# deepsound-project/pggan-pytorch

Hardware: AMD Instinct MI355X
Metric: images/sec, PGGAN full train step (D+GP step + G step + Adam) at 1024x1024 (higher is better)
Workload: dtype f32; 1 GPU; BASELINE config 5: PGGAN 1024x1024 net (fmap_base 4096, C=3, latent 512), stage depth 8 = 1024x1024, alpha 1.00, minibatch 3/GPU (reference schedule), Trainer.train(): WGAN-GP + Adam(0,0.99) at lr 0, fp32; resolution=1024, depth=8, minibatch_per_gpu=3, global_batch=3, parallelism=dp1, fmap_base=4096, hip_graphs=False

## Files before the change

pggan-pytorch_amd/csrc/conv_strip.hip:

```cpp
#include "convp.h"

#ifndef PG_STRIP_ABL
#define PG_STRIP_ABL 0
#endif

namespace {

using pgk::ConvP;
using pgk::pg_sign_byte;
using pgk::pg_sign_factors;
using pgk::g_last_kernel; using pgk::set_smem; using pgk::SMEM_ANY;

constexpr int SW = 64;
constexpr int RP = SW + 2;
constexpr int RB = 4;
constexpr int NBLK = 3;

enum { EPI_GENERIC = 0, EPI_FWD = 1, EPI_MASK = 2, EPI_PN = 3, EPI_PNB = 4 };

struct SArgs {
    const float* x; const float* w; const float* bias; const void* mask; float* y;
    unsigned char* ysigns; float* pn_r; const float* pnb_y; const float* pnb_r; float* ypool; const float* pool_other;
    float scale, slope, mask_slope, pn_eps, pool_a, pool_b;
    int H, W, ups, mask_bytes, y_bytes, pool_only;
    int strips, segs, seg_rows;
    const unsigned char* gbytes; float gmul, gslope;
    const float* rgb_w; const float* rgb_b; float rgb_scale, rgb_slope; int rgbC; unsigned char* xsigns;
    float* t_out; const float* t_w; const float* t_b; float t_scale; int tC, t_sc, t_sco, t_only;
    const float* fw_img; float* fw_dw; float* fw_db; float fw_scale;
};

template <int CIN> struct Blk {
    static constexpr int C4 = CIN / 4;
    static constexpr int USED = C4 * RB * RP;
    static constexpr int NWI = (USED + 63) / 64;
    static constexpr int NI = (NWI + 3) / 4;
    static constexpr int SLOTS = NWI * 64;
};

typedef __attribute__((address_space(3))) const char* lds_cptr;
typedef __attribute__((address_space(3))) const f32x4* lds_v4ptr;

__device__ __forceinline__ pg_u32x4 rsrc_words(const void* base, unsigned bytes)
{
    const unsigned long long a = (unsigned long long)base;
    return pg_u32x4{(unsigned)__builtin_amdgcn_readfirstlane((int)(unsigned)a),
                    (unsigned)__builtin_amdgcn_readfirstlane((int)((unsigned)(a >> 32) & 0xffffu)), bytes, 0x00020000u};
}
__device__ __forceinline__ void buf_store4(__amdgpu_buffer_rsrc_t r, unsigned voff, float4 v)
{
    __builtin_amdgcn_raw_buffer_store_b128(pg_u32x4{__float_as_uint(v.x), __float_as_uint(v.y), __float_as_uint(v.z), __float_as_uint(v.w)},
                                           r, (int)voff, 0, 0);
}

constexpr int RGB_MAXC = 3;
template <int COUT, int CIN, int EPI, bool WREG, int GM, int XM = 0>
__device__ __forceinline__ void conv_strip_body(const SArgs& p)
{
    constexpr bool GATH = GM != 0;
    using B = Blk<CIN>;
    constexpr int C4 = B::C4;
    constexpr int QO = COUT / 4, QP = 16 / QO, PXG = 4 * QP;
    constexpr int GPR = 32 / PXG, G = 2 * GPR;
    constexpr int BLKB = B::SLOTS * 16;
    constexpr bool GEN = EPI == EPI_GENERIC;
    extern __shared__ __align__(16) float lds[];
    constexpr int WS = CIN == 16 ? CIN + 4 : CIN;
    float* wl = lds + NBLK * B::SLOTS * 4;
    const int tid = threadIdx.x, lane = tid & 63, wave = __builtin_amdgcn_readfirstlane(tid >> 6);
    const int blk = lane >> 2, j = lane & 3, qo = blk % QO, qp = blk / QO;

    int t = (int)pg_xcd_remap(blockIdx.x, gridDim.x);
    const int strip = __builtin_amdgcn_readfirstlane(t % p.strips); t /= p.strips;
    const int seg = __builtin_amdgcn_readfirstlane(t % p.segs), n = __builtin_amdgcn_readfirstlane(t / p.segs);
    const int r0 = seg * p.seg_rows, ow0 = strip * SW;
    const int niter = p.seg_rows / RB;
    const int xH = p.ups ? (p.H >> 1) : p.H, xW = p.ups ? (p.W >> 1) : p.W;
    const unsigned npix = (unsigned)(p.H * p.W);

    const unsigned rowbytes = 4u * (unsigned)(xW * CIN);
    unsigned voff[B::NI], vstep[B::NI];
    const unsigned blkstep = (p.ups ? 2u : 4u) * rowbytes;
#pragma unroll
    for (int i = 0; i < B::NI; ++i) {
        const int sl = (i * 4 + wave) * 64 + lane;
        const int q = sl / (RB * RP), rem = sl - q * (RB * RP);
        const int m = rem / RP, px = rem - m * RP;
        const int col = ow0 - 1 + px, row = r0 - 1 + m;
        const bool ok = sl < B::USED && (unsigned)col < (unsigned)p.W;
        voff[i] = ok ? (unsigned)(p.ups ? (row >> 1) : row) * rowbytes + 4u * (unsigned)((p.ups ? (col >> 1) : col) * CIN + 4 * q) : PG_OOB;
        vstep[i] = ok ? blkstep : 0u;
    }
    const size_t ximg = (size_t)xH * xW * CIN;
    const pg_u32x4 rxs = rsrc_words(p.x + (size_t)n * ximg, (unsigned)(ximg * 4));
    const unsigned lds0 = (unsigned)(size_t)(__attribute__((address_space(3))) char*)lds;
    const unsigned wdst = __builtin_amdgcn_readfirstlane(lds0 + (unsigned)wave * 1024u);
    auto dma16 = [&](unsigned vo, unsigned dst) {
        unsigned keep;
        asm volatile("s_mov_b32 %0, m0\n\ts_mov_b32 m0, %3\n\ts_nop 0\n\tbuffer_load_dwordx4 %1, %2, 0 offen lds\n\ts_mov_b32 m0, %0"
                     : "=&s"(keep) : "v"(vo), "s"(rxs), "s"(dst) : "memory");
    };
    auto issue_block = [&](int pos) {
#pragma unroll
        for (int i = 0; i < B::NI; ++i) {
            if (i * 4 + wave < B::NWI) dma16(voff[i], wdst + (unsigned)pos * BLKB + (unsigned)i * 4096u);
            voff[i] += vstep[i];
        }
    };

    constexpr int NG = GATH ? (B::USED + 255) / 256 : 1;
    unsigned cvo[NG], cvs[NG], bvo[NG], bvs[NG];
    float4 gxr[NG];
    unsigned gbr[NG];
    __amdgpu_buffer_rsrc_t rgx = pg_make_rsrc(p.x + (size_t)n * ximg, (unsigned)(ximg * 4)), rgb = rgx;
    constexpr int NR = GM == 2 ? NG : 1;
    int rrow[NR];
    float rw[NR][4][RGB_MAXC], rb[NR][4], rpx[NR][RGB_MAXC];
    if constexpr (GM == 2) {
        rgx = pg_make_rsrc(p.x + (size_t)n * npix * p.rgbC, npix * (unsigned)p.rgbC * 4u);
        rgb = pg_make_rsrc(p.xsigns + (size_t)n * npix * C4, npix * C4);
#pragma unroll
        for (int i = 0; i < NG; ++i) {
            const int sl = i * 256 + tid;
            const int q = sl / (RB * RP), rem = sl - q * (RB * RP);
            const int m = rem / RP, px = rem - m * RP;
            const int col = ow0 - 1 + px;
            const bool ok = sl < B::USED && (unsigned)col < (unsigned)p.W;
            rrow[i] = ok ? r0 - 1 + m : -(1 << 28);
            cvo[i] = ok ? 4u * (unsigned)((r0 - 1 + m) * p.W + col) : PG_OOB;
            cvs[i] = ok ? 4u * (unsigned)(RB * p.W) : 0u;
            bvo[i] = (ok && px >= 1 && px <= SW) ? (unsigned)((r0 - 1 + m) * p.W + col) * C4 + q : PG_OOB;
            bvs[i] = (ok && px >= 1 && px <= SW) ? (unsigned)(RB * p.W * C4) : 0u;
            const int qq = sl < B::USED ? q : 0;
#pragma unroll
            for (int k = 0; k < 4; ++k) {
#pragma unroll
                for (int c = 0; c < RGB_MAXC; ++c) rw[i][k][c] = c < p.rgbC ? p.rgb_w[(4 * qq + k) * p.rgbC + c] : 0.f;
                rb[i][k] = p.rgb_b ? p.rgb_b[4 * qq + k] : 0.f;
            }
        }
    }
    if constexpr (GM == 1) {
        rgb = pg_make_rsrc(p.gbytes + (size_t)n * npix * C4, npix * C4);
#pragma unroll
        for (int i = 0; i < NG; ++i) {
            const int sl = i * 256 + tid;
            const int q = sl / (RB * RP), rem = sl - q * (RB * RP);
            const int m = rem / RP, px = rem - m * RP;
            const int col = ow0 - 1 + px, row = r0 - 1 + m;
            const bool ok = sl < B::USED && (unsigned)col < (unsigned)p.W;
            cvo[i] = ok ? (unsigned)(row >> 1) * rowbytes + 4u * (unsigned)((col >> 1) * CIN + 4 * q) : PG_OOB;
            cvs[i] = ok ? 2u * rowbytes : 0u;
            bvo[i] = ok ? (unsigned)(row * p.W + col) * C4 + q : PG_OOB;
            bvs[i] = ok ? (unsigned)(RB * p.W * C4) : 0u;
        }
    }
    auto gather_load = [&]() {
        if constexpr (GM == 2) {
#pragma unroll
            for (int i = 0; i < NG; ++i) {
                const bool in = (unsigned)rrow[i] < (unsigned)p.H;
#pragma unroll
                for (int c = 0; c < RGB_MAXC; ++c)
                    rpx[i][c] = c < p.rgbC ? __uint_as_float(__builtin_amdgcn_raw_buffer_load_b32(rgx, in ? (int)(cvo[i] + (unsigned)c * npix * 4u) : (int)PG_OOB, 0, 0)) : 0.f;
                cvo[i] += cvs[i];
            }
            return;
        }
#pragma unroll
        for (int i = 0; i < NG; ++i) {
            gxr[i] = pg_buf_load4(rgx, cvo[i], 0);
            gbr[i] = __builtin_amdgcn_raw_buffer_load_b8(rgb, (int)bvo[i], 0, 0);
            cvo[i] += cvs[i]; bvo[i] += bvs[i];
        }
    };
    auto gather_store = [&](int pos) {
        if constexpr (GM == 2) {
#pragma unroll
            for (int i = 0; i < NG; ++i) {
                const int sl = i * 256 + tid;
                const bool in = (unsigned)rrow[i] < (unsigned)p.H;
                float o[4];
#pragma unroll
                for (int k = 0; k < 4; ++k) {
                    float a = 0.f;
#pragma unroll
                    for (int c = 0; c < RGB_MAXC; ++c) if (c < p.rgbC) a = fmaf(rpx[i][c], rw[i][k][c], a);
                    const float v = __fadd_rn(__fmul_rn(a, p.rgb_scale), rb[i][k]);
                    o[k] = in ? (v > 0.f ? v : v * p.rgb_slope) : 0.f;
                }
                const float4 v4 = make_float4(o[0], o[1], o[2], o[3]);
                if (sl < B::SLOTS) *reinterpret_cast<float4*>(lds + (pos * B::SLOTS + sl) * 4) = (cvs[i] ? v4 : make_float4(0.f, 0.f, 0.f, 0.f));
                if (p.xsigns && in && rrow[i] >= r0 && rrow[i] < r0 + p.seg_rows && bvs[i])
                    __builtin_amdgcn_raw_buffer_store_b8(pg_sign_byte(v4), rgb, (int)bvo[i], 0, 0);
                bvo[i] += bvs[i];
                rrow[i] += RB;
            }
            return;
        }
#pragma unroll
        for (int i = 0; i < NG; ++i) {
            const int sl = i * 256 + tid;
            if (sl < B::SLOTS) {
                const float4 f = pg_sign_factors((unsigned char)gbr[i], p.gslope);
                const float4 v = gxr[i];
                *reinterpret_cast<float4*>(lds + (pos * B::SLOTS + sl) * 4) =
                    make_float4(v.x * (f.x * p.gmul), v.y * (f.y * p.gmul), v.z * (f.z * p.gmul), v.w * (f.w * p.gmul));
            }
        }
    };

    float4 wreg[WREG ? 9 : 1][WREG ? C4 : 1];
    if constexpr (WREG) {
#pragma unroll
        for (int tp = 0; tp < 9; ++tp)
#pragma unroll
            for (int c4 = 0; c4 < C4; ++c4)
                wreg[tp][c4] = *reinterpret_cast<const float4*>(p.w + ((size_t)(tp * COUT + 4 * qo + j) * CIN + 4 * c4));
    } else {
        for (int e = tid; e < 9 * COUT * C4; e += 256)
            *reinterpret_cast<float4*>(wl + (e / C4) * WS + 4 * (e % C4)) = *reinterpret_cast<const float4*>(p.w + 4 * e);
    }
    const float* wrow = wl + (4 * qo + j) * WS;

    if constexpr (GATH) {
        gather_load(); gather_store(0);
        gather_load(); gather_store(1);
    } else {
        issue_block(0);
        issue_block(1);
    }

    const int rp = wave >> 1;
    const int col0 = (wave & 1) * 32;
    const lds_cptr lbase = (lds_cptr)lds + (col0 + 4 * qp + j) * 16;

    const bool has_mask = (GEN && p.mask) || EPI == EPI_MASK;
    const bool mask_bytes = has_mask && p.mask_bytes;
    const bool has_pnb = (GEN && p.pnb_y) || EPI == EPI_PNB;
    const bool has_pn = (GEN && p.pn_r) || EPI == EPI_PN;
    const bool has_signs = (GEN || EPI == EPI_FWD) && p.ysigns;
    const bool has_pool = GEN && p.ypool;
    const bool y_bytes = GEN && p.y_bytes;
    const bool has_trgb = (XM & 1) != 0 && (EPI == EPI_PN || EPI == EPI_MASK) && p.t_out != nullptr;
    const bool has_fw = (XM & 2) != 0 && EPI == EPI_MASK && COUT == 8 && p.fw_dw != nullptr;
    const bool y_store = !(has_pool && p.pool_only) && !y_bytes && !((has_trgb || has_fw) && p.t_only);
    const __amdgpu_buffer_rsrc_t ry = y_bytes ? pg_make_rsrc((const unsigned char*)p.y + (size_t)n * npix * (COUT / 4), npix * (COUT / 4))
                                              : pg_make_rsrc(p.y + (size_t)n * npix * COUT, npix * COUT * 4u);
    __amdgpu_buffer_rsrc_t rmask = ry, rsig = ry, rpnr = ry, rpnby = ry, rpnbr = ry;
    if (has_mask) rmask = mask_bytes ? pg_make_rsrc((const unsigned char*)p.mask + (size_t)n * npix * (COUT / 4), npix * (COUT / 4))
                                     : pg_make_rsrc((const float*)p.mask + (size_t)n * npix * COUT, npix * COUT * 4u);
    if (has_signs) rsig = pg_make_rsrc(p.ysigns + (size_t)n * npix * (COUT / 4), npix * (COUT / 4));
    if (has_pn) rpnr = pg_make_rsrc(p.pn_r + (size_t)n * npix, npix * 4u);
    if (has_pnb) {
        rpnby = pg_make_rsrc(p.pnb_y + (size_t)n * npix * COUT, npix * COUT * 4u);
        rpnbr = pg_make_rsrc(p.pnb_r + (size_t)n * npix, npix * 4u);
    }
    const unsigned pix0 = (unsigned)((r0 + 2 * rp) * p.W + ow0 + col0 + 4 * qp + j);
    float4 bv = make_float4(0.f, 0.f, 0.f, 0.f);
    if (!has_mask && p.bias) bv = *reinterpret_cast<const float4*>(p.bias + 4 * qo);
    float tw[RGB_MAXC][4], tb[RGB_MAXC];
    float aw[4][RGB_MAXC], ab[4], fi[G][RGB_MAXC];
#pragma unroll
    for (int k = 0; k < 4; ++k) {
        ab[k] = 0.f;
#pragma unroll
        for (int c = 0; c < RGB_MAXC; ++c) aw[k][c] = 0.f;
    }
    __amdgpu_buffer_rsrc_t rfimg = ry;
    if (has_fw) rfimg = pg_make_rsrc(p.fw_img + (size_t)n * npix * p.tC, npix * (unsigned)p.tC * 4u);
    __amdgpu_buffer_rsrc_t rtout = ry;
    if (has_trgb) {
        rtout = pg_make_rsrc(p.t_out + (size_t)n * npix * p.tC, npix * (unsigned)p.tC * 4u);
#pragma unroll
        for (int c = 0; c < RGB_MAXC; ++c) {
#pragma unroll
            for (int k = 0; k < 4; ++k) tw[c][k] = c < p.tC ? p.t_w[c * p.t_sc + (4 * qo + k) * p.t_sco] : 0.f;
            tb[c] = (c < p.tC && p.t_b) ? p.t_b[c] : 0.f;
        }
    }

    f32x4 acc[G], acc2[G];
    auto compute = [&](auto ph_, auto rp_) {
        constexpr int PH = decltype(ph_)::value, RPAIR = decltype(rp_)::value;
#pragma unroll
        for (int g = 0; g < G; ++g) { acc[g] = f32x4{0.f, 0.f, 0.f, 0.f}; acc2[g] = f32x4{0.f, 0.f, 0.f, 0.f}; }
#pragma unroll
        for (int tp = 0; tp < ((PG_STRIP_ABL & 4) ? 1 : 9); ++tp) {
            const int dy = tp / 3, dx = tp % 3;
#pragma unroll
            for (int c4 = 0; c4 < C4; ++c4) {
                float4 a;
                if constexpr (WREG) a = wreg[tp][c4];
                else a = *reinterpret_cast<const float4*>(wrow + tp * COUT * WS + 4 * c4);
                f32x4 bq[G];
#pragma unroll
                for (int g = 0; g < G; ++g) {
                    const int m = 2 * RPAIR + g / GPR + dy;
                    const int pos = m < RB ? PH : (PH + 1) % NBLK;
                    const int off = ((pos * B::SLOTS) + c4 * (RB * RP) + (m & (RB - 1)) * RP + (g % GPR) * PXG + dx) * 16;
                    bq[g] = *(lds_v4ptr)(lbase + off);
                }
#pragma unroll
                for (int g = 0; g < G; ++g) acc[g] = __builtin_amdgcn_mfma_f32_4x4x1f32(a.x, bq[g][0], acc[g], 0, 0, 0);
#pragma unroll
                for (int g = 0; g < G; ++g) acc2[g] = __builtin_amdgcn_mfma_f32_4x4x1f32(a.y, bq[g][1], acc2[g], 0, 0, 0);
#pragma unroll
                for (int g = 0; g < G; ++g) acc[g] = __builtin_amdgcn_mfma_f32_4x4x1f32(a.z, bq[g][2], acc[g], 0, 0, 0);
#pragma unroll
                for (int g = 0; g < G; ++g) acc2[g] = __builtin_amdgcn_mfma_f32_4x4x1f32(a.w, bq[g][3], acc2[g], 0, 0, 0);
            }
        }
#pragma unroll
        for (int g = 0; g < G; ++g) acc[g] += acc2[g];
    };

    float4 pm[G];
    unsigned pmb[G];
    float prr[G];
    auto prefetch_epilogue = [&](unsigned pix) {
#pragma unroll
        for (int g = 0; g < G; ++g) {
            const unsigned pg_ = pix + (unsigned)((g / GPR) * p.W + (g % GPR) * PXG);
            if (has_fw) {
#pragma unroll
                for (int c = 0; c < RGB_MAXC; ++c)
                    fi[g][c] = c < p.tC ? __uint_as_float(__builtin_amdgcn_raw_buffer_load_b32(rfimg, (int)(((unsigned)c * npix + pg_) * 4u), 0, 0)) : 0.f;
            }
            if (has_mask) {
                if (mask_bytes) pmb[g] = __builtin_amdgcn_raw_buffer_load_b8(rmask, (int)(pg_ * (COUT / 4) + qo), 0, 0);
                else pm[g] = pg_buf_load4(rmask, (pg_ * COUT + 4 * qo) * 4u, 0);
            } else if (has_pnb) {
                pm[g] = pg_buf_load4(rpnby, (pg_ * COUT + 4 * qo) * 4u, 0);
                prr[g] = __uint_as_float(__builtin_amdgcn_raw_buffer_load_b32(rpnbr, (int)(pg_ * 4u), 0, 0));
            }
        }
    };
    auto epilogue = [&](unsigned pix) {
        float4 ov[G];
#pragma unroll
        for (int g = 0; g < G; ++g) {
            const unsigned pg_ = pix + (unsigned)((g / GPR) * p.W + (g % GPR) * PXG);
            const unsigned off = pg_ * COUT + 4 * qo;
            float4 o = make_float4(acc[g][0] * p.scale, acc[g][1] * p.scale, acc[g][2] * p.scale, acc[g][3] * p.scale);
            if (has_mask) {
                float4 f;
                if (mask_bytes) f = pg_sign_factors((unsigned char)pmb[g], p.mask_slope);
                else {
                    const float4 mk = pm[g];
                    f = make_float4(mk.x > 0.f ? 1.f : p.mask_slope, mk.y > 0.f ? 1.f : p.mask_slope,
                                    mk.z > 0.f ? 1.f : p.mask_slope, mk.w > 0.f ? 1.f : p.mask_slope);
                }
                o.x *= f.x; o.y *= f.y; o.z *= f.z; o.w *= f.w;
            } else {
                o.x += bv.x; o.y += bv.y; o.z += bv.z; o.w += bv.w;
                o.x = o.x > 0.f ? o.x : o.x * p.slope; o.y = o.y > 0.f ? o.y : o.y * p.slope;
                o.z = o.z > 0.f ? o.z : o.z * p.slope; o.w = o.w > 0.f ? o.w : o.w * p.slope;
                if (has_signs && !(PG_STRIP_ABL & 2)) __builtin_amdgcn_raw_buffer_store_b8(pg_sign_byte(o), rsig, (int)(off >> 2), 0, 0);
            }
            if (has_pnb) {
                const float4 yv = pm[g];
                const float4 gv = make_float4(acc[g][0] * p.scale, acc[g][1] * p.scale, acc[g][2] * p.scale, acc[g][3] * p.scale);
                float dt = (gv.x * yv.x + gv.y * yv.y) + (gv.z * yv.z + gv.w * yv.w);
                dt += __shfl_xor(dt, 4, 64);
                if (QO >= 4) dt += __shfl_xor(dt, 8, 64);
                const float rr = prr[g], mean = dt / (float)COUT;
                o.x = rr * (gv.x - yv.x * mean) * (yv.x > 0.f ? 1.f : p.mask_slope);
                o.y = rr * (gv.y - yv.y * mean) * (yv.y > 0.f ? 1.f : p.mask_slope);
                o.z = rr * (gv.z - yv.z * mean) * (yv.z > 0.f ? 1.f : p.mask_slope);
                o.w = rr * (gv.w - yv.w * mean) * (yv.w > 0.f ? 1.f : p.mask_slope);
            }
            if (has_pn) {
                float ssq = (o.x * o.x + o.y * o.y) + (o.z * o.z + o.w * o.w);
                ssq += __shfl_xor(ssq, 4, 64);
                if (QO >= 4) ssq += __shfl_xor(ssq, 8, 64);
                const float rr = rsqrtf(ssq / (float)COUT + p.pn_eps);
                o.x *= rr; o.y *= rr; o.z *= rr; o.w *= rr;
                if (qo == 0 && !(PG_STRIP_ABL & 2)) __builtin_amdgcn_raw_buffer_store_b32(__float_as_uint(rr), rpnr, (int)(pg_ * 4u), 0, 0);
            }
            if (has_fw) {
                const float ov4[4] = {o.x, o.y, o.z, o.w};
#pragma unroll
                for (int k = 0; k < 4; ++k) {
                    ab[k] += ov4[k];
#pragma unroll
                    for (int c = 0; c < RGB_MAXC; ++c) aw[k][c] = fmaf(ov4[k], fi[g][c], aw[k][c]);
                }
            }
            if (has_trgb) {
#pragma unroll
                for (int c = 0; c < RGB_MAXC; ++c) {
                    if (c >= p.tC) break;
                    float a = fmaf(o.w, tw[c][3], fmaf(o.z, tw[c][2], fmaf(o.y, tw[c][1], o.x * tw[c][0])));
                    a += __shfl_xor(a, 4, 64);
                    if (QO >= 4) a += __shfl_xor(a, 8, 64);
                    if (qo == 0) __builtin_amdgcn_raw_buffer_store_b32(__float_as_uint(fmaf(a, p.t_scale, tb[c])), rtout, (int)(((unsigned)c * npix + pg_) * 4u), 0, 0);
                }
            }
            if (!(PG_STRIP_ABL & 2)) {
                if (y_bytes) __builtin_amdgcn_raw_buffer_store_b8(pg_sign_byte(o), ry, (int)(off >> 2), 0, 0);
                else if (y_store) buf_store4(ry, off * 4u, o);
            }
            ov[g] = o;
        }
        if (has_pool) {
#pragma unroll
            for (int g = 0; g < G; ++g) {
                ov[g].x += __shfl_xor(ov[g].x, 1, 64); ov[g].y += __shfl_xor(ov[g].y, 1, 64);
                ov[g].z += __shfl_xor(ov[g].z, 1, 64); ov[g].w += __shfl_xor(ov[g].w, 1, 64);
            }
#pragma unroll
            for (int g = 0; g < GPR; ++g) {
                float4 v = make_float4((ov[g].x + ov[g + GPR].x) * 0.25f, (ov[g].y + ov[g + GPR].y) * 0.25f,
                                       (ov[g].z + ov[g + GPR].z) * 0.25f, (ov[g].w + ov[g + GPR].w) * 0.25f);
                if (j & 1) continue;
                const unsigned pg_ = pix + (unsigned)(g * PXG);
                const unsigned oy = pg_ / (unsigned)p.W, ox = pg_ - oy * (unsigned)p.W;
                const size_t poff = (((size_t)n * (p.H >> 1) + (oy >> 1)) * (p.W >> 1) + (ox >> 1)) * COUT + 4 * qo;
                if (p.pool_other) {
                    const float4 q = *reinterpret_cast<const float4*>(p.pool_other + poff);
                    v.x = fmaf(v.x, p.pool_a, p.pool_b * q.x); v.y = fmaf(v.y, p.pool_a, p.pool_b * q.y);
                    v.z = fmaf(v.z, p.pool_a, p.pool_b * q.z); v.w = fmaf(v.w, p.pool_a, p.pool_b * q.w);
                } else if (p.pool_a != 1.f) { v.x *= p.pool_a; v.y *= p.pool_a; v.z *= p.pool_a; v.w *= p.pool_a; }
                *reinterpret_cast<float4*>(p.ypool + poff) = v;
            }
        }
    };

    int nstores = (y_bytes || y_store) ? G : 0;
    if (has_signs) nstores += G;
    if (has_pn) nstores += G;
    if (has_pool) nstores += GPR;
    if (has_trgb) nstores += G * p.tC;
    if (PG_STRIP_ABL & 2) nstores = 0;
    nstores = __builtin_amdgcn_readfirstlane(nstores);
    auto wait_dma = [&]() {
        if constexpr (EPI == EPI_MASK || EPI == EPI_PNB || EPI == EPI_PN) {
            static_assert(G == 2, "");
            if (!has_trgb && !has_fw) {
                if constexpr (EPI == EPI_PN) asm volatile("s_waitcnt vmcnt(4)" ::: "memory");
                else asm volatile("s_waitcnt vmcnt(2)" ::: "memory");
            } else switch (nstores) {
                case 2: asm volatile("s_waitcnt vmcnt(2)" ::: "memory"); break;
                case 4: asm volatile("s_waitcnt vmcnt(4)" ::: "memory"); break;
                case 6: asm volatile("s_waitcnt vmcnt(6)" ::: "memory"); break;
                case 8: asm volatile("s_waitcnt vmcnt(8)" ::: "memory"); break;
                case 10: asm volatile("s_waitcnt vmcnt(10)" ::: "memory"); break;
                default: asm volatile("s_waitcnt vmcnt(0)" ::: "memory"); break;
            }
        }
        else switch (nstores) {
            case 0: asm volatile("s_waitcnt vmcnt(0)" ::: "memory"); break;
            case 1: asm volatile("s_waitcnt vmcnt(1)" ::: "memory"); break;
            case 2: asm volatile("s_waitcnt vmcnt(2)" ::: "memory"); break;
            case 3: asm volatile("s_waitcnt vmcnt(3)" ::: "memory"); break;
            case 4: asm volatile("s_waitcnt vmcnt(4)" ::: "memory"); break;
            case 5: asm volatile("s_waitcnt vmcnt(5)" ::: "memory"); break;
            default: asm volatile("s_waitcnt vmcnt(6)" ::: "memory"); break;
        }
    };
    unsigned pix = pix0;
    const unsigned pixstep = (unsigned)(RB * p.W);
    auto step = [&](int it, auto ph_) {
        constexpr int PH = decltype(ph_)::value;
        if constexpr (!GATH) {
            if (it == 0 || (PG_STRIP_ABL & 2)) asm volatile("s_waitcnt vmcnt(0)" ::: "memory");
            else wait_dma();
        }
        __syncthreads();
        const bool more = it + 2 <= niter;
        if constexpr (GATH) { if (more) gather_load(); }
        else if (more && !((PG_STRIP_ABL & 1) && it > 0)) issue_block((PH + 2) % NBLK);
        prefetch_epilogue(pix);
        __builtin_amdgcn_sched_barrier(0);
        if (rp == 0) compute(ph_, std::integral_constant<int, 0>{});
        else compute(ph_, std::integral_constant<int, 1>{});
        if constexpr (GATH) { if (more) gather_store((PH + 2) % NBLK); }
        epilogue(pix);
        pix += pixstep;
    };
    for (int it = 0; it < niter; it += 3) {
        step(it, std::integral_constant<int, 0>{});
        if (it + 1 < niter) step(it + 1, std::integral_constant<int, 1>{});
        if (it + 2 < niter) step(it + 2, std::integral_constant<int, 2>{});
    }
    if (has_fw) {
        static_assert(COUT != 8 || QO == 2, "");
        float v[16];
#pragma unroll
        for (int k = 0; k < 4; ++k) {
#pragma unroll
            for (int c = 0; c < RGB_MAXC; ++c) v[4 * k + c] = aw[k][c];
            v[4 * k + 3] = ab[k];
        }
#pragma unroll
        for (int i = 0; i < 16; ++i) {
            float a = v[i];
            a += __shfl_xor(a, 1, 64); a += __shfl_xor(a, 2, 64); a += __shfl_xor(a, 8, 64); a += __shfl_xor(a, 16, 64); a += __shfl_xor(a, 32, 64);
            v[i] = a;
        }
        __syncthreads();
        if ((lane & ~4) == 0) {
#pragma unroll
            for (int i = 0; i < 16; ++i) lds[(wave * 2 + (lane >> 2)) * 16 + i] = v[i];
        }
        __syncthreads();
        const int q2 = (tid >> 4) & 1, i = tid & 15, k = i >> 2, c = i & 3, co = 4 * q2 + k;
        auto commit = [&](float a) {
            if (c < 3) { if (c < p.tC) atomicAdd(p.fw_dw + co * p.tC + c, a * p.fw_scale); }
            else if (p.fw_db) atomicAdd(p.fw_db + co, a);
        };
        float a = 0.f;
        if (tid < 32) a = (lds[(0 * 2 + q2) * 16 + i] + lds[(1 * 2 + q2) * 16 + i]) + (lds[(2 * 2 + q2) * 16 + i] + lds[(3 * 2 + q2) * 16 + i]);
        if (tid < 32) commit(a);
    }
}

template <int COUT, int CIN, int EPI, bool WREG, bool GATH>
__global__ __launch_bounds__(256, GATH ? 2 : (WREG ? 3 : 4)) void conv_strip_kernel(SArgs p)
{
    conv_strip_body<COUT, CIN, EPI, WREG, GATH ? 1 : 0>(p);
}

template <int EPI, bool WREG, int XM>
__global__ __launch_bounds__(256, 3) void conv_strip_x_kernel(SArgs p)
{
    conv_strip_body<8, 8, EPI, WREG, 0, XM>(p);
}

template <int EPI>
__global__ __launch_bounds__(256, 2) void conv_strip_rgb_kernel(SArgs p)
{
    conv_strip_body<8, 8, EPI, false, 2>(p);
}

template <int COUT, int CIN, int EPI, bool WREG, bool GATH = false>
int launch_strip(const SArgs& a, int N, hipStream_t s)
{
    using B = Blk<CIN>;
    const size_t smem = (size_t)NBLK * B::SLOTS * 16 + (WREG ? 0 : (size_t)9 * COUT * (CIN == 16 ? CIN + 4 : CIN) * 4);
    auto kern = conv_strip_kernel<COUT, CIN, EPI, WREG, GATH>;
    if (int rc = set_smem(kern, smem, SMEM_ANY)) return rc;
    snprintf(g_last_kernel, sizeof(g_last_kernel), "conv_strip_kernel<%d, %d, %d, %s, %s>", COUT, CIN, EPI, WREG ? "true" : "false", GATH ? "true" : "false");
    hipLaunchKernelGGL(kern, dim3((unsigned)(N * a.strips * a.segs)), dim3(256), smem, s, a);
    return (int)hipGetLastError();
}

template <int EPI, bool WREG, int XM>
int launch_strip_x(const SArgs& a, int N, hipStream_t s)
{
    const size_t smem = (size_t)NBLK * Blk<8>::SLOTS * 16 + (WREG ? 0 : (size_t)9 * 8 * 8 * 4);
    auto kern = conv_strip_x_kernel<EPI, WREG, XM>;
    if (int rc = set_smem(kern, smem, SMEM_ANY)) return rc;
    snprintf(g_last_kernel, sizeof(g_last_kernel), "conv_strip_x_kernel<%d, %s, %d>", EPI, WREG ? "true" : "false", XM);
    hipLaunchKernelGGL(kern, dim3((unsigned)(N * a.strips * a.segs)), dim3(256), smem, s, a);
    return (int)hipGetLastError();
}

template <int COUT, int CIN, bool WREG>
int launch_strip_epi(const SArgs& a, int epi, int N, hipStream_t s)
{
    switch (epi) {
        case EPI_FWD: return launch_strip<COUT, CIN, EPI_FWD, WREG>(a, N, s);
        case EPI_MASK: return launch_strip<COUT, CIN, EPI_MASK, WREG>(a, N, s);
        case EPI_PN: return launch_strip<COUT, CIN, EPI_PN, WREG>(a, N, s);
        case EPI_PNB: return launch_strip<COUT, CIN, EPI_PNB, WREG>(a, N, s);
        default: return launch_strip<COUT, CIN, EPI_GENERIC, WREG>(a, N, s);
    }
}

struct WArgs { const float* x; const float* gz; float* dw; float* db; float scale; int H, W, ups, strips, segs, seg_rows;
               const unsigned char* gbytes; float gmul, gslope; };

template <int CO, int CI, bool GATH>
__global__ __launch_bounds__(256, 2) void wgrad_strip_kernel(WArgs p)
{
    constexpr int TAPS = 9;
    constexpr int QO = CO / 4, QI = CI / 4, NB = QO * QI, PPM = 16 / NB, RNG = SW / PPM;
    static_assert(NB == 4 || NB == 8, "8x8, 16x8 or 8x16 channels");
    constexpr int XU = RNG + 2, XRS = PPM * XU;
    constexpr int XBS = 320, GBS = RB * SW;
    static_assert(RB * XRS <= XBS, "");
    constexpr int XRING = 3, GRING = 2;
    constexpr int XPS = XRING * XBS + 2, GPS = GRING * GBS + 2;
    constexpr int XNWI = QI * 5, GNWI = QO * RB, XNI = (XNWI + 3) / 4, GNI = (GNWI + 3) / 4;
    extern __shared__ __align__(16) float lds[];
    const unsigned lds0 = (unsigned)(size_t)(__attribute__((address_space(3))) char*)lds;
    constexpr unsigned GLDS = (unsigned)QI * XPS * 16;
    const int tid = threadIdx.x, lane = tid & 63, wave = __builtin_amdgcn_readfirstlane(tid >> 6);
    const int blk = lane >> 2, i4 = lane & 3;
    const int hi = blk % QI, ho = (blk / QI) % QO, slot = blk / NB;

    int t = (int)pg_xcd_remap(blockIdx.x, gridDim.x);
    const int strip = __builtin_amdgcn_readfirstlane(t % p.strips); t /= p.strips;
    const int seg = __builtin_amdgcn_readfirstlane(t % p.segs), n = __builtin_amdgcn_readfirstlane(t / p.segs);
    const int r0 = seg * p.seg_rows, ow0 = strip * SW;
    const int niter = p.seg_rows / RB;
    const int xH = p.ups ? (p.H >> 1) : p.H, xW = p.ups ? (p.W >> 1) : p.W;

    const unsigned xrowbytes = 4u * (unsigned)(xW * CI), grow = 4u * (unsigned)(p.W * CO);
    unsigned xvoff[XNI], xvstep[XNI], xdst[XNI], gvoff[GNI], gdst[GNI];
    const unsigned xblkstep = (p.ups ? 2u : 4u) * xrowbytes;
#pragma unroll
    for (int i = 0; i < XNI; ++i) {
        const int ii = i * 4 + wave, q = ii / 5, part = ii - q * 5;
        const int idx = part * 64 + lane;
        const int m = idx / XRS, e = idx - m * XRS, u = e / PPM, s = e - u * PPM;
        const int col = ow0 + RNG * s + u - 1, row = r0 - 1 + m;
        const bool ok = ii < XNWI && idx < RB * XRS && (unsigned)col < (unsigned)p.W;
        xvoff[i] = ok ? (unsigned)(p.ups ? (row >> 1) : row) * xrowbytes + 4u * (unsigned)((p.ups ? (col >> 1) : col) * CI + 4 * q) : PG_OOB;
        xvstep[i] = ok ? xblkstep : 0u;
        xdst[i] = lds0 + (unsigned)(q * XPS + part * 64) * 16u;
    }
#pragma unroll
    for (int i = 0; i < GNI; ++i) {
        const int jj = i * 4 + wave, q = jj / RB, m = jj - q * RB;
        const int u = lane / PPM, s = lane - u * PPM;
        const int col = ow0 + RNG * s + u, row = r0 + m;
        gvoff[i] = jj < GNWI ? (unsigned)row * grow + 4u * (unsigned)(col * CO + 4 * q) : PG_OOB;
        gdst[i] = lds0 + GLDS + (unsigned)(q * GPS + m * SW) * 16u;
    }
    const size_t ximg = (size_t)xH * xW * CI, gimg = GATH ? (size_t)(p.H >> 1) * (p.W >> 1) * CO : (size_t)p.H * p.W * CO;
    const pg_u32x4 rxs = rsrc_words(p.x + (size_t)n * ximg, (unsigned)(ximg * 4));
    const pg_u32x4 rgs = rsrc_words(p.gz + (size_t)n * gimg, (unsigned)(gimg * 4));
    constexpr int NGZ = GATH ? QO : 1;
    unsigned cvo[NGZ], bvo[NGZ];
    float4 gxr[NGZ];
    unsigned gbr[NGZ];
    __amdgpu_buffer_rsrc_t rgc = pg_make_rsrc(p.gz + (size_t)n * gimg, (unsigned)(gimg * 4)), rgb = rgc;
    if constexpr (GATH) {
        rgb = pg_make_rsrc(p.gbytes + (size_t)n * p.H * p.W * QO, (unsigned)(p.H * p.W * QO));
        const int m = tid >> 6, e = tid & 63, u = e / PPM, s = e - u * PPM;
        const int col = ow0 + RNG * s + u, row = r0 + m;
#pragma unroll
        for (int q = 0; q < NGZ; ++q) {
            cvo[q] = 4u * (unsigned)(((row >> 1) * (p.W >> 1) + (col >> 1)) * CO + 4 * q);
            bvo[q] = (unsigned)(row * p.W + col) * QO + q;
        }
    }
    auto gather_load = [&]() {
#pragma unroll
        for (int q = 0; q < NGZ; ++q) {
            gxr[q] = pg_buf_load4(rgc, cvo[q], 0);
            gbr[q] = __builtin_amdgcn_raw_buffer_load_b8(rgb, (int)bvo[q], 0, 0);
            cvo[q] += 2u * 4u * (unsigned)((p.W >> 1) * CO); bvo[q] += (unsigned)(RB * p.W * QO);
        }
    };
    auto gather_store = [&](int pos) {
#pragma unroll
        for (int q = 0; q < NGZ; ++q) {
            const float4 f = pg_sign_factors((unsigned char)gbr[q], p.gslope);
            const float4 v = gxr[q];
            *reinterpret_cast<float4*>(lds + GLDS / 4 + ((q * GPS + pos * GBS) + tid) * 4) =
                make_float4(v.x * (f.x * p.gmul), v.y * (f.y * p.gmul), v.z * (f.z * p.gmul), v.w * (f.w * p.gmul));
        }
    };
    auto dma16 = [&](const pg_u32x4& rs, unsigned vo, unsigned dst) {
        unsigned keep;
        asm volatile("s_mov_b32 %0, m0\n\ts_mov_b32 m0, %3\n\ts_nop 0\n\tbuffer_load_dwordx4 %1, %2, 0 offen lds\n\ts_mov_b32 m0, %0"
                     : "=&s"(keep) : "v"(vo), "s"(rs), "s"(dst) : "memory");
    };
    auto issue_x = [&](int pos) {
#pragma unroll
        for (int i = 0; i < XNI; ++i) {
            if (i * 4 + wave < XNWI) dma16(rxs, xvoff[i], __builtin_amdgcn_readfirstlane(xdst[i]) + (unsigned)pos * (XBS * 16u));
            xvoff[i] += xvstep[i];
        }
    };
    auto issue_g = [&](int pos) {
#pragma unroll
        for (int i = 0; i < GNI; ++i) {
            if (i * 4 + wave < GNWI) dma16(rgs, gvoff[i], __builtin_amdgcn_readfirstlane(gdst[i]) + (unsigned)pos * (GBS * 16u));
            gvoff[i] += 4u * grow;
        }
    };
    issue_x(0);
    if constexpr (GATH) { gather_load(); gather_store(0); } else issue_g(0);
    issue_x(1);

    f32x4 acc[TAPS];
#pragma unroll
    for (int tp = 0; tp < TAPS; ++tp) acc[tp] = f32x4{0.f, 0.f, 0.f, 0.f};
    float bsum = 0.f;
    typedef __attribute__((address_space(3))) const float* lds_fptr;
    const lds_cptr xl = (lds_cptr)lds + (hi * XPS + slot) * 16 + i4 * 4;
    const lds_cptr gl = (lds_cptr)lds + GLDS + (ho * GPS + slot) * 16 + i4 * 4;

    for (int it = 0; it < niter; ++it) {
        asm volatile("s_waitcnt vmcnt(0)" ::: "memory");
        __syncthreads();
        if (it + 2 <= niter) issue_x((it + 2) % XRING);
        if constexpr (GATH) { if (it + 1 < niter) gather_load(); }
        else if (it + 1 < niter) issue_g((it + 1) % GRING);
        __builtin_amdgcn_sched_barrier(0);
        const int rr0 = (RB * (it % XRING) + wave);
        lds_cptr xb[3];
#pragma unroll
        for (int dy = 0; dy < 3; ++dy) {
            int rr = rr0 + dy; if (rr >= RB * XRING) rr -= RB * XRING;
            xb[dy] = xl + ((rr / RB) * XBS + (rr % RB) * XRS) * 16;
        }
        const lds_cptr gb = gl + ((it % GRING) * GBS + wave * SW) * 16;
        float bcol[3][3];
#pragma unroll
        for (int dy = 0; dy < 3; ++dy) {
            bcol[dy][0] = *(lds_fptr)(xb[dy] + 0 * PPM * 16);
            bcol[dy][1] = *(lds_fptr)(xb[dy] + 1 * PPM * 16);
        }
#pragma unroll
        for (int ks = 0; ks < RNG; ++ks) {
            const float a = *(lds_fptr)(gb + ks * PPM * 16);
#pragma unroll
            for (int dy = 0; dy < 3; ++dy) bcol[dy][(ks + 2) % 3] = *(lds_fptr)(xb[dy] + (ks + 2) * PPM * 16);
            bsum += a;
#pragma unroll
            for (int dy = 0; dy < 3; ++dy)
#pragma unroll
                for (int dx = 0; dx < 3; ++dx)
                    acc[dy * 3 + dx] = __builtin_amdgcn_mfma_f32_4x4x1f32(a, bcol[dy][(ks + dx) % 3], acc[dy * 3 + dx], 0, 0, 0);
        }
        if constexpr (GATH) { if (it + 1 < niter) gather_store((it + 1) % GRING); }
    }

#pragma unroll
    for (int tp = 0; tp < TAPS; ++tp)
#pragma unroll
        for (int r = 0; r < 4; ++r) {
            float v = acc[tp][r];
            v += __shfl_xor(v, 32, 64);
            if (PPM >= 4) v += __shfl_xor(v, 16, 64);
            acc[tp][r] = v;
        }
    bsum += __shfl_xor(bsum, 32, 64);
    if (PPM >= 4) bsum += __shfl_xor(bsum, 16, 64);
    constexpr int NL = 4 * NB, NE = TAPS * 4 + 1;
    __syncthreads();
    float* red = lds;
    if (lane < NL) {
#pragma unroll
        for (int tp = 0; tp < TAPS; ++tp)
#pragma unroll
            for (int r = 0; r < 4; ++r) red[(wave * NE + tp * 4 + r) * NL + lane] = acc[tp][r];
        red[(wave * NE + TAPS * 4) * NL + lane] = bsum;
    }
    __syncthreads();
    for (int e = tid; e < NE * NL; e += 256) {
        const int l = e % NL, ve = e / NL;
        const float v = (red[e] + red[e + NE * NL]) + (red[e + 2 * NE * NL] + red[e + 3 * NE * NL]);
        const int b_ = l >> 2, jj = l & 3;
        const int hi_ = b_ % QI, ho_ = (b_ / QI) % QO;
        if (ve < TAPS * 4) {
            const int tp = ve >> 2, r = ve & 3;
            atomicAdd(p.dw + ((size_t)(tp * CO + 4 * ho_ + r) * CI + 4 * hi_ + jj), v * p.scale);
        } else if (p.db && hi_ == 0) {
            atomicAdd(p.db + 4 * ho_ + jj, v);
        }
    }
}

template <int CO, int CI, bool GATH = false>
int launch_wgrad_strip_t(const WArgs& a, int N, hipStream_t s)
{
    constexpr int QO = CO / 4, QI = CI / 4;
    const size_t smem = ((size_t)QI * (3 * 320 + 2) + (size_t)QO * (2 * RB * SW + 2)) * 16;
    auto kern = wgrad_strip_kernel<CO, CI, GATH>;
    if (int rc = set_smem(kern, smem, SMEM_ANY)) return rc;
    snprintf(g_last_kernel, sizeof(g_last_kernel), "wgrad_strip_kernel<%d, %d, %s>", CO, CI, GATH ? "true" : "false");
    hipLaunchKernelGGL(kern, dim3((unsigned)(N * a.strips * a.segs)), dim3(256), smem, s, a);
    return (int)hipGetLastError();
}

int strip_seg_rows(int N, int H, int W)
{
    int seg = 64;
    while (seg > 16 && ((long long)N * (W / SW) * (H / seg) < 768 || (H % seg))) seg >>= 1;
    return (seg < 16 || (seg % RB) || (H % seg)) ? 0 : seg;
}

constexpr bool STRIP_WREG = true;

}

int pgk::launch_conv_strip(ConvP& p, hipStream_t s)
{
    if (p.KS != 3 || p.pad != 1 || p.yup || p.ksplit != 1) return PG_E_UNSUP;
    if ((p.Wout % SW) || (p.Hout % 16) || p.Hout != p.Hin || p.Wout != p.Win) return PG_E_UNSUP;
    if (!(p.Cout == 8 && (p.Cin == 8 || p.Cin == 16))) return PG_E_UNSUP;
    if ((long long)p.Hin * p.Win * 16 * 4 >= (1ll << 31)) return PG_E_UNSUP;
    const int seg = strip_seg_rows(p.N, p.Hout, p.Wout);
    if (!seg) return PG_E_UNSUP;
    SArgs a{};
    a.x = p.x; a.w = p.w; a.bias = p.bias; a.mask = p.mask; a.y = p.y;
    a.ysigns = p.ysigns; a.pn_r = p.pn_r; a.pnb_y = p.pnb_y; a.pnb_r = p.pnb_r; a.ypool = p.ypool; a.pool_other = p.pool_other;
    a.scale = p.scale; a.slope = p.slope; a.mask_slope = p.mask_slope; a.pn_eps = p.pn_eps; a.pool_a = p.pool_a; a.pool_b = p.pool_b;
    a.H = p.Hout; a.W = p.Wout; a.ups = p.ups; a.mask_bytes = p.mask_bytes; a.y_bytes = p.y_bytes; a.pool_only = p.pool_only;
    a.strips = p.Wout / SW; a.segs = p.Hout / seg; a.seg_rows = seg;
    a.gbytes = p.gbytes; a.gmul = p.gmul; a.gslope = p.gslope;
    if (p.gbytes) {
        if (!p.ups || p.bias || p.ypool || p.y_bytes || p.pnb_y || p.pn_r || p.ysigns) return PG_E_UNSUP;
        if (p.Cin == 8) return p.mask ? launch_strip<8, 8, EPI_MASK, false, true>(a, p.N, s)
                                      : launch_strip<8, 8, EPI_FWD, false, true>(a, p.N, s);
        return p.mask ? launch_strip<8, 16, EPI_MASK, false, true>(a, p.N, s)
                      : launch_strip<8, 16, EPI_FWD, false, true>(a, p.N, s);
    }
    int epi = EPI_GENERIC;
    if (!p.ypool && !p.y_bytes) {
        if (p.pnb_y && !p.mask && !p.pn_r && !p.ysigns) epi = EPI_PNB;
        else if (p.pn_r && !p.mask && !p.pnb_y && !p.ysigns) epi = EPI_PN;
        else if (p.mask && !p.pnb_y && !p.pn_r) epi = EPI_MASK;
        else if (!p.mask && !p.pnb_y && !p.pn_r) epi = EPI_FWD;
    }
    if (p.Cin == 8) return launch_strip_epi<8, 8, STRIP_WREG>(a, epi, p.N, s);
    return launch_strip_epi<8, 16, false>(a, epi, p.N, s);
}

int pgk::launch_conv_strip_fromrgb(const float* img, const float* rgb_w, const float* rgb_b, float rgb_scale, float rgb_slope,
                                   unsigned char* x_signs, const float* w, const float* bias, float* y, unsigned char* y_signs,
                                   int N, int C, int H, int W, int Cmid, int Cout, float scale, float slope,
                                   hipStream_t s)
{
    if (C > RGB_MAXC || Cmid != 8 || Cout != 8 || (W % SW) || (H % 16)) return PG_E_UNSUP;
    if ((long long)H * W * 16 * 4 >= (1ll << 31)) return PG_E_UNSUP;
    const int seg = strip_seg_rows(N, H, W);
    if (!seg) return PG_E_UNSUP;
    SArgs a{};
    a.x = img; a.w = w; a.bias = bias; a.y = y; a.ysigns = y_signs;
    a.scale = scale; a.slope = slope; a.mask_slope = 1.f; a.pool_a = 1.f;
    a.H = H; a.W = W; a.strips = W / SW; a.segs = H / seg; a.seg_rows = seg;
    a.rgb_w = rgb_w; a.rgb_b = rgb_b; a.rgb_scale = rgb_scale; a.rgb_slope = rgb_slope; a.rgbC = C; a.xsigns = x_signs;
    const size_t smem = (size_t)NBLK * Blk<8>::SLOTS * 16 + (size_t)9 * 8 * 8 * 4;
    auto kern = conv_strip_rgb_kernel<EPI_FWD>;
    if (int rc = set_smem(kern, smem, SMEM_ANY)) return rc;
    snprintf(g_last_kernel, sizeof(g_last_kernel), "conv_strip_rgb_kernel<%d>", (int)EPI_FWD);
    hipLaunchKernelGGL(kern, dim3((unsigned)(N * a.strips * a.segs)), dim3(256), smem, s, a);
    return (int)hipGetLastError();
}

int pgk::launch_conv_strip_pn_torgb(const float* x, const float* w, const float* bias, float* y, float* r,
                                    const float* t_w, const float* t_b, float t_scale, float* img,
                                    int N, int C, int H, int W, int Cin, int Cout, float scale, float slope, float eps,
                                    hipStream_t s)
{
    if (C < 1 || C > RGB_MAXC || Cin != 8 || Cout != 8 || (W % SW) || (H % 16)) return PG_E_UNSUP;
    if ((long long)H * W * 16 * 4 >= (1ll << 31)) return PG_E_UNSUP;
    const int seg = strip_seg_rows(N, H, W);
    if (!seg) return PG_E_UNSUP;
    SArgs a{};
    a.x = x; a.w = w; a.bias = bias; a.y = y; a.pn_r = r; a.pn_eps = eps;
    a.scale = scale; a.slope = slope; a.mask_slope = 1.f; a.pool_a = 1.f;
    a.H = H; a.W = W; a.strips = W / SW; a.segs = H / seg; a.seg_rows = seg;
    a.t_out = img; a.t_w = t_w; a.t_b = t_b; a.t_scale = t_scale; a.tC = C; a.t_sc = Cout; a.t_sco = 1;
    return launch_strip_x<EPI_PN, STRIP_WREG, 1>(a, N, s);
}

int pgk::launch_conv_strip_masked_rgb_bwd(const float* gz, const float* wt, const unsigned char* mask_bytes, float mask_slope, float* y,
                                          const float* rgb_w, float rgb_scale, float* gimg,
                                          const float* img, float* rgb_dw, float* rgb_db,
                                          int N, int C, int H, int W, int Cin, int Cout, float scale,
                                          hipStream_t s)
{
    if (C < 1 || C > RGB_MAXC || Cin != 8 || Cout != 8 || (W % SW) || (H % 16)) return PG_E_UNSUP;
    if ((long long)H * W * 16 * 4 >= (1ll << 31)) return PG_E_UNSUP;
    const int seg = strip_seg_rows(N, H, W);
    if (!seg) return PG_E_UNSUP;
    SArgs a{};
    a.x = gz; a.w = wt; a.mask = mask_bytes; a.mask_bytes = 1; a.y = y;
    a.scale = scale; a.slope = 1.f; a.mask_slope = mask_slope; a.pool_a = 1.f;
    a.H = H; a.W = W; a.strips = W / SW; a.segs = H / seg; a.seg_rows = seg;
    a.t_out = gimg; a.t_w = rgb_w; a.t_b = nullptr; a.t_scale = rgb_scale; a.tC = C; a.t_sc = 1; a.t_sco = C; a.t_only = y ? 0 : 1;
    a.fw_img = img; a.fw_dw = rgb_dw; a.fw_db = rgb_db; a.fw_scale = rgb_scale;
    if (rgb_dw) return launch_strip_x<EPI_MASK, false, 3>(a, N, s);
    return launch_strip_x<EPI_MASK, false, 1>(a, N, s);
}

int pgk::launch_wgrad_strip(WgP& p, hipStream_t s)
{
    if (p.pad != 1 || p.Hout != p.Hin || p.Wout != p.Win || (p.gbytes && p.ups)) return PG_E_UNSUP;
    if ((p.Wout % SW) || (p.Hout % 16)) return PG_E_UNSUP;
    if (!((p.Cout == 8 && p.Cin == 8) || (p.Cout == 16 && p.Cin == 8) || (p.Cout == 8 && p.Cin == 16))) return PG_E_UNSUP;
    if ((long long)p.Hin * p.Win * 16 * 4 >= (1ll << 31)) return PG_E_UNSUP;
    int seg = 256;
    auto tasks = [&](int sg) { return (long long)p.N * (p.Wout / SW) * (p.Hout / sg); };
    while (seg > 64 && (seg > p.Hout || (p.Hout % seg) || tasks(seg) < 1024)) seg >>= 1;
    while (seg > 16 && (seg > p.Hout || (p.Hout % seg) || tasks(seg) < 512)) seg >>= 1;
    if (seg < 16 || (seg % RB) || (p.Hout % seg)) return PG_E_UNSUP;
    WArgs a;
    a.x = p.x; a.gz = p.gz; a.dw = p.dw; a.db = p.db; a.scale = p.scale;
    a.H = p.Hout; a.W = p.Wout; a.ups = p.ups; a.strips = p.Wout / SW; a.segs = p.Hout / seg; a.seg_rows = seg;
    a.gbytes = p.gbytes; a.gmul = p.gmul; a.gslope = p.gslope;
    if (p.gbytes) {
        if (p.Cout == 8 && p.Cin == 8) return launch_wgrad_strip_t<8, 8, true>(a, p.N, s);
        if (p.Cout == 16 && p.Cin == 8) return launch_wgrad_strip_t<16, 8, true>(a, p.N, s);
        return launch_wgrad_strip_t<8, 16, true>(a, p.N, s);
    }
    if (p.Cout == 8 && p.Cin == 8) return launch_wgrad_strip_t<8, 8>(a, p.N, s);
    if (p.Cout == 16 && p.Cin == 8) return launch_wgrad_strip_t<16, 8>(a, p.N, s);
    return launch_wgrad_strip_t<8, 16>(a, p.N, s);
}
```

Before: 300.2 images/sec.

## Remap strip-conv gather so each lane loads one pixel's full channel vector

Replaces the slot-indexed gather, where each thread handled scattered (channel-quad,row,col) slots, with a pixel-major mapping: each wave owns one row, each lane one interior column and loads all channel quads plus packed sign bytes in wider loads. Halo columns are handled by one rotating wave per step, and unused LDS slots are zeroed once up front. The goal is to coalesce global loads, cut per-thread index bookkeeping and registers, and widen sign stores. It also adds ablation macros that skip gather work. Risks are halo-wave imbalance and LDS bank conflicts from the new write pattern.

```diff
diff --git a/pggan-pytorch_amd/csrc/conv_strip.hip b/pggan-pytorch_amd/csrc/conv_strip.hip
--- a/pggan-pytorch_amd/csrc/conv_strip.hip
+++ b/pggan-pytorch_amd/csrc/conv_strip.hip
@@ -108,106 +108,138 @@
         }
     };
 
-    constexpr int NG = GATH ? (B::USED + 255) / 256 : 1;
-    unsigned cvo[NG], cvs[NG], bvo[NG], bvs[NG];
-    float4 gxr[NG];
-    unsigned gbr[NG];
     __amdgpu_buffer_rsrc_t rgx = pg_make_rsrc(p.x + (size_t)n * ximg, (unsigned)(ximg * 4)), rgb = rgx;
-    constexpr int NR = GM == 2 ? NG : 1;
-    int rrow[NR];
-    float rw[NR][4][RGB_MAXC], rb[NR][4], rpx[NR][RGB_MAXC];
-    if constexpr (GM == 2) {
-        rgx = pg_make_rsrc(p.x + (size_t)n * npix * p.rgbC, npix * (unsigned)p.rgbC * 4u);
-        rgb = pg_make_rsrc(p.xsigns + (size_t)n * npix * C4, npix * C4);
-#pragma unroll
-        for (int i = 0; i < NG; ++i) {
-            const int sl = i * 256 + tid;
-            const int q = sl / (RB * RP), rem = sl - q * (RB * RP);
-            const int m = rem / RP, px = rem - m * RP;
-            const int col = ow0 - 1 + px;
-            const bool ok = sl < B::USED && (unsigned)col < (unsigned)p.W;
-            rrow[i] = ok ? r0 - 1 + m : -(1 << 28);
-            cvo[i] = ok ? 4u * (unsigned)((r0 - 1 + m) * p.W + col) : PG_OOB;
-            cvs[i] = ok ? 4u * (unsigned)(RB * p.W) : 0u;
-            bvo[i] = (ok && px >= 1 && px <= SW) ? (unsigned)((r0 - 1 + m) * p.W + col) * C4 + q : PG_OOB;
-            bvs[i] = (ok && px >= 1 && px <= SW) ? (unsigned)(RB * p.W * C4) : 0u;
-            const int qq = sl < B::USED ? q : 0;
+    constexpr int HL = GM == 2 ? 2 * RB : 2 * RB * C4;
+    unsigned cvo = 0, bvo = 0, cstep = 0, bstep = 0;
+    unsigned hcvo = PG_OOB, hcs = 0, hbvo = PG_OOB, hbs = 0;
+    int grow = r0 - 1 + wave, hrow = -(1 << 28);
+    int hslot = 0, gturn = 0;
+    float4 gxr[C4], hxr = make_float4(0.f, 0.f, 0.f, 0.f);
+    unsigned gbr = 0, hbr = 0;
+    constexpr int NRW = GM == 2 ? 8 : 1;
+    float rw[NRW][RGB_MAXC], rb[NRW], rpx[RGB_MAXC] = {0.f, 0.f, 0.f}, hpx[RGB_MAXC] = {0.f, 0.f, 0.f};
+    if constexpr (GATH) {
+        const int hp = GM == 2 ? lane : lane / C4, hq = GM == 2 ? 0 : lane % C4;
+        const int hm = (hp >> 1) & (RB - 1), hpxl = (hp & 1) ? RP - 1 : 0;
+        const int hcol = ow0 - 1 + hpxl, hr = r0 - 1 + hm, icol = ow0 + lane;
+        const bool hok = lane < HL && (unsigned)hcol < (unsigned)p.W;
+        hslot = hq * (RB * RP) + hm * RP + hpxl;
+        if constexpr (GM == 2) {
+            rgx = pg_make_rsrc(p.x + (size_t)n * npix * p.rgbC, npix * (unsigned)p.rgbC * 4u);
+            rgb = pg_make_rsrc(p.xsigns + (size_t)n * npix * C4, npix * C4);
+            cvo = 4u * (unsigned)(grow * p.W + icol);
+            cstep = 4u * (unsigned)(RB * p.W);
+            bvo = (unsigned)(grow * p.W + icol) * C4;
+            bstep = (unsigned)(RB * p.W * C4);
+            hcvo = hok ? 4u * (unsigned)(hr * p.W + hcol) : PG_OOB;
+            hcs = hok ? cstep : 0u;
+            hrow = hok ? hr : -(1 << 28);
+#pragma unroll
+            for (int k = 0; k < NRW; ++k) {
+#pragma unroll
+                for (int c = 0; c < RGB_MAXC; ++c) rw[k][c] = c < p.rgbC ? p.rgb_w[k * p.rgbC + c] : 0.f;
+                rb[k] = p.rgb_b ? p.rgb_b[k] : 0.f;
+            }
+        } else {
+            rgb = pg_make_rsrc(p.gbytes + (size_t)n * npix * C4, npix * C4);
+            cvo = (unsigned)(grow >> 1) * rowbytes + 4u * (unsigned)((icol >> 1) * CIN);
+            cstep = 2u * rowbytes;
+            bvo = (unsigned)(grow * p.W + icol) * C4;
+            bstep = (unsigned)(RB * p.W * C4);
+            hcvo = hok ? (unsigned)(hr >> 1) * rowbytes + 4u * (unsigned)((hcol >> 1) * CIN + 4 * hq) : PG_OOB;
+            hcs = hok ? cstep : 0u;
+            hbvo = hok ? (unsigned)(hr * p.W + hcol) * C4 + hq : PG_OOB;
+            hbs = hok ? bstep : 0u;
+        }
+        if (tid < B::SLOTS - B::USED) {
+#pragma unroll
+            for (int pos = 0; pos < NBLK; ++pos)
+                *reinterpret_cast<float4*>(lds + (pos * B::SLOTS + B::USED + tid) * 4) = make_float4(0.f, 0.f, 0.f, 0.f);
+        }
+    }
+    auto rgb_pixel = [&](const float (&px)[RGB_MAXC], bool in, float4 (&o)[2]) {
+#pragma unroll
+        for (int q = 0; q < 2; ++q) {
+            float t[4];
 #pragma unroll
             for (int k = 0; k < 4; ++k) {
-#pragma unroll
-                for (int c = 0; c < RGB_MAXC; ++c) rw[i][k][c] = c < p.rgbC ? p.rgb_w[(4 * qq + k) * p.rgbC + c] : 0.f;
-                rb[i][k] = p.rgb_b ? p.rgb_b[4 * qq + k] : 0.f;
-            }
-        }
-    }
-    if constexpr (GM == 1) {
-        rgb = pg_make_rsrc(p.gbytes + (size_t)n * npix * C4, npix * C4);
-#pragma unroll
-        for (int i = 0; i < NG; ++i) {
-            const int sl = i * 256 + tid;
-            const int q = sl / (RB * RP), rem = sl - q * (RB * RP);
-            const int m = rem / RP, px = rem - m * RP;
-            const int col = ow0 - 1 + px, row = r0 - 1 + m;
-            const bool ok = sl < B::USED && (unsigned)col < (unsigned)p.W;
-            cvo[i] = ok ? (unsigned)(row >> 1) * rowbytes + 4u * (unsigned)((col >> 1) * CIN + 4 * q) : PG_OOB;
-            cvs[i] = ok ? 2u * rowbytes : 0u;
-            bvo[i] = ok ? (unsigned)(row * p.W + col) * C4 + q : PG_OOB;
-            bvs[i] = ok ? (unsigned)(RB * p.W * C4) : 0u;
-        }
-    }
+                const int co = GM == 2 ? 4 * q + k : 0;
+                float a = 0.f;
+#pragma unroll
+                for (int c = 0; c < RGB_MAXC; ++c) if (c < p.rgbC) a = fmaf(px[c], rw[co][c], a);
+                const float v = __fadd_rn(__fmul_rn(a, p.rgb_scale), rb[co]);
+                t[k] = in ? (v > 0.f ? v : v * p.rgb_slope) : 0.f;
+            }
+            o[q] = make_float4(t[0], t[1], t[2], t[3]);
+        }
+    };
     auto gather_load = [&]() {
+        const bool turn = (gturn & 3) == wave;
         if constexpr (GM == 2) {
-#pragma unroll
-            for (int i = 0; i < NG; ++i) {
-                const bool in = (unsigned)rrow[i] < (unsigned)p.H;
+            const bool in = (unsigned)grow < (unsigned)p.H, hin = (unsigned)hrow < (unsigned)p.H;
+#pragma unroll
+            for (int c = 0; c < RGB_MAXC; ++c)
+                rpx[c] = c < p.rgbC ? __uint_as_float(__builtin_amdgcn_raw_buffer_load_b32(rgx, in ? (int)(cvo + (unsigned)c * npix * 4u) : (int)PG_OOB, 0, 0)) : 0.f;
+            if (turn) {
 #pragma unroll
                 for (int c = 0; c < RGB_MAXC; ++c)
-                    rpx[i][c] = c < p.rgbC ? __uint_as_float(__builtin_amdgcn_raw_buffer_load_b32(rgx, in ? (int)(cvo[i] + (unsigned)c * npix * 4u) : (int)PG_OOB, 0, 0)) : 0.f;
-                cvo[i] += cvs[i];
-            }
+                    hpx[c] = c < p.rgbC ? __uint_as_float(__builtin_amdgcn_raw_buffer_load_b32(rgx, hin ? (int)(hcvo + (unsigned)c * npix * 4u) : (int)PG_OOB, 0, 0)) : 0.f;
+            }
+            cvo += cstep; hcvo += hcs;
             return;
         }
 #pragma unroll
-        for (int i = 0; i < NG; ++i) {
-            gxr[i] = pg_buf_load4(rgx, cvo[i], 0);
-            gbr[i] = __builtin_amdgcn_raw_buffer_load_b8(rgb, (int)bvo[i], 0, 0);
-            cvo[i] += cvs[i]; bvo[i] += bvs[i];
-        }
-    };
+        for (int q = 0; q < C4; ++q) gxr[q] = pg_buf_load4(rgx, cvo + 16u * (unsigned)q, 0);
+        if constexpr (C4 == 4) gbr = __builtin_amdgcn_raw_buffer_load_b32(rgb, (int)bvo, 0, 0);
+        else gbr = __builtin_amdgcn_raw_buffer_load_b16(rgb, (int)bvo, 0, 0);
+        if (turn) {
+            hxr = pg_buf_load4(rgx, hcvo, 0);
+            hbr = __builtin_amdgcn_raw_buffer_load_b8(rgb, (int)hbvo, 0, 0);
+        }
+        cvo += cstep; bvo += bstep; hcvo += hcs; hbvo += hbs;
+    };
+    const bool ring_wr = !(PG_STRIP_ABL & 16) || p.seg_rows < 0;
     auto gather_store = [&](int pos) {
+        const bool turn = (gturn & 3) == wave;
+        float* const ring = lds + pos * (B::SLOTS * 4);
+        float* const dst = ring + (wave * RP + lane + 1) * 4;
         if constexpr (GM == 2) {
-#pragma unroll
-            for (int i = 0; i < NG; ++i) {
-                const int sl = i * 256 + tid;
-                const bool in = (unsigned)rrow[i] < (unsigned)p.H;
-                float o[4];
-#pragma unroll
-                for (int k = 0; k < 4; ++k) {
-                    float a = 0.f;
-#pragma unroll
-                    for (int c = 0; c < RGB_MAXC; ++c) if (c < p.rgbC) a = fmaf(rpx[i][c], rw[i][k][c], a);
-                    const float v = __fadd_rn(__fmul_rn(a, p.rgb_scale), rb[i][k]);
-                    o[k] = in ? (v > 0.f ? v : v * p.rgb_slope) : 0.f;
+            const bool in = (unsigned)grow < (unsigned)p.H;
+            float4 o[2];
+            rgb_pixel(rpx, in, o);
+            if (ring_wr) {
+                *reinterpret_cast<float4*>(dst) = o[0];
+                *reinterpret_cast<float4*>(dst + RB * RP * 4) = o[1];
+            }
+            if (p.xsigns && in && grow >= r0 && grow < r0 + p.seg_rows)
+                __builtin_amdgcn_raw_buffer_store_b16((unsigned short)(pg_sign_byte(o[0]) | (pg_sign_byte(o[1]) << 8)), rgb, (int)bvo, 0, 0);
+            if (turn) {
+                rgb_pixel(hpx, (unsigned)hrow < (unsigned)p.H, o);
+                if (lane < HL && ring_wr) {
+                    *reinterpret_cast<float4*>(ring + hslot * 4) = o[0];
+                    *reinterpret_cast<float4*>(ring + (hslot + RB * RP) * 4) = o[1];
                 }
-                const float4 v4 = make_float4(o[0], o[1], o[2], o[3]);
-                if (sl < B::SLOTS) *reinterpret_cast<float4*>(lds + (pos * B::SLOTS + sl) * 4) = (cvs[i] ? v4 : make_float4(0.f, 0.f, 0.f, 0.f));
-                if (p.xsigns && in && rrow[i] >= r0 && rrow[i] < r0 + p.seg_rows && bvs[i])
-                    __builtin_amdgcn_raw_buffer_store_b8(pg_sign_byte(v4), rgb, (int)bvo[i], 0, 0);
-                bvo[i] += bvs[i];
-                rrow[i] += RB;
-            }
+            }
+            bvo += bstep; grow += RB; hrow += RB;
+            ++gturn;
             return;
         }
-#pragma unroll
-        for (int i = 0; i < NG; ++i) {
-            const int sl = i * 256 + tid;
-            if (sl < B::SLOTS) {
-                const float4 f = pg_sign_factors((unsigned char)gbr[i], p.gslope);
-                const float4 v = gxr[i];
-                *reinterpret_cast<float4*>(lds + (pos * B::SLOTS + sl) * 4) =
+        if (ring_wr) {
+#pragma unroll
+            for (int q = 0; q < C4; ++q) {
+                const float4 f = pg_sign_factors((unsigned char)(gbr >> (8 * q)), p.gslope);
+                const float4 v = gxr[q];
+                *reinterpret_cast<float4*>(dst + q * (RB * RP * 4)) =
                     make_float4(v.x * (f.x * p.gmul), v.y * (f.y * p.gmul), v.z * (f.z * p.gmul), v.w * (f.w * p.gmul));
             }
-        }
+            if (turn && lane < HL) {
+                const float4 f = pg_sign_factors((unsigned char)hbr, p.gslope);
+                const float4 v = hxr;
+                *reinterpret_cast<float4*>(ring + hslot * 4) =
+                    make_float4(v.x * (f.x * p.gmul), v.y * (f.y * p.gmul), v.z * (f.z * p.gmul), v.w * (f.w * p.gmul));
+            }
+        }
+        ++gturn;
     };
 
     float4 wreg[WREG ? 9 : 1][WREG ? C4 : 1];
@@ -469,13 +501,13 @@
         }
         __syncthreads();
         const bool more = it + 2 <= niter;
-        if constexpr (GATH) { if (more) gather_load(); }
+        if constexpr (GATH) { if (more && !((PG_STRIP_ABL & (8 | 32)) && it > 0)) gather_load(); }
         else if (more && !((PG_STRIP_ABL & 1) && it > 0)) issue_block((PH + 2) % NBLK);
         prefetch_epilogue(pix);
         __builtin_amdgcn_sched_barrier(0);
         if (rp == 0) compute(ph_, std::integral_constant<int, 0>{});
         else compute(ph_, std::integral_constant<int, 1>{});
-        if constexpr (GATH) { if (more) gather_store((PH + 2) % NBLK); }
+        if constexpr (GATH) { if (more && !((PG_STRIP_ABL & 32) && it > 0)) gather_store((PH + 2) % NBLK); }
         epilogue(pix);
         pix += pixstep;
     };
```

Result: no change. 301.1 images/sec, median of 3 (+0.3%).
